# MarcBerliner/PETLION.jl

Hardware: AMD Instinct MI355X
Metric: DFN full-discharge trajectories/sec (ensemble) (higher is better)
Workload: dtype f64

## Files before the change

### petlion.jl_amd/csrc/dfn_cell.h

```cpp
#pragma once
#include <hip/hip_runtime.h>
#include <type_traits>
#include "../../include/petlion_hip.h"

namespace pl {

#ifndef PL_DEV
#define PL_DEV __device__ inline
#endif

constexpr int WAVE = 64;
#ifndef PL_NP
#define PL_NP 10
#endif
#ifndef PL_NS
#define PL_NS 10
#endif
#ifndef PL_NN
#define PL_NN 10
#endif
#ifndef PL_NR
#define PL_NR 10
#endif
#ifndef PL_NRN
// ... 275 lines not shown
#elif defined(PL_PHASE_FENCES) && !defined(PL_PHASE_TIMERS) && !defined(PL_WAVE_EMU)
#define PL_FENCE_() __asm__ volatile("" ::: "memory")
#define PL_AMARK(txt) PL_FENCE_()
#define PL_TIC() PL_FENCE_()
#define PL_TOC(S_, ph) PL_FENCE_()
#define PL_TIC_TOTAL() do {} while (0)
#define PL_TOC_TOTAL(S_) do {} while (0)
#define PL_TICD() PL_FENCE_()
#define PL_TOCD(S_, slot) PL_FENCE_()
#define PL_TICE(mode) PL_FENCE_()
#define PL_TOCE(S_, mode, slot) PL_FENCE_()
#else
#define PL_TIC() PL_TIC_()
#define PL_TOC(S_, ph) PL_TOC_(S_, ph)
#define PL_TIC_TOTAL() do {} while (0)
#define PL_TOC_TOTAL(S_) PL_TOC_(S_, PH_TOTAL)
#define PL_TICD() do {} while (0)
#define PL_TOCD(S_, slot) do {} while (0)
#define PL_TICE(mode) do {} while (0)
#define PL_TOCE(S_, mode, slot) do {} while (0)
#endif
#ifndef PL_AMARK
#define PL_AMARK(txt) do {} while (0)
#endif
__host__ __device__ __forceinline__ int sec_of(int i) { return i < NP ? 0 : (i < NP + NS ? 1 : 2); }
#ifndef PL_WAVE_EMU
template <int CTRL> __device__ __forceinline__ double dpp_mov0(double v) {
  int lo = __double2loint(v), hi = __double2hiint(v);
  lo = __builtin_amdgcn_update_dpp(0, lo, CTRL, 0xf, 0xf, true);
  hi = __builtin_amdgcn_update_dpp(0, hi, CTRL, 0xf, 0xf, true);
  return __hiloint2double(hi, lo);
}
__device__ __forceinline__ double shift_up1(double v) { return dpp_mov0<0x138>(v); }
__device__ __forceinline__ double shift_down1(double v) { return dpp_mov0<0x130>(v); }
__device__ __forceinline__ double row_up2(double v) { return dpp_mov0<0x112>(v); }
__device__ __forceinline__ double row_down2(double v) { return dpp_mov0<0x102>(v); }
__device__ __forceinline__ double lane_bcast(double v, int src) {
  const int lo = __builtin_amdgcn_readlane(__double2loint(v), src), hi = __builtin_amdgcn_readlane(__double2hiint(v), src);
  return __hiloint2double(hi, lo);
}
__device__ __forceinline__ int lane_bcast_i(int v, int src) { return __builtin_amdgcn_readlane(v, src); }
__device__ __forceinline__ double wave_sum(double v) {
  v += dpp_mov0<0x111>(v); v += dpp_mov0<0x112>(v); v += dpp_mov0<0x114>(v); v += dpp_mov0<0x118>(v);
  return (lane_bcast(v, 15) + lane_bcast(v, 31)) + (lane_bcast(v, 47) + lane_bcast(v, 63));
}
#else
// ... 1429 lines not shown
```

### petlion.jl_amd/csrc/dfn_integrate.h

```cpp
#pragma once
#include "dfn_cell.h"

namespace pl {

constexpr int NTRIP_MAX = (2 * NE + NJ * NR + 2 * NJ + 1 + (NT > 2 * NN + 1 ? NT : 2 * NN + 1) + WAVE - 1) / WAVE;
struct IdaScalars {
  double tn, hh, hused, cj, cjlast, cjold, cjratio, ss, rr, h0_forced, rtol, atol;
  double ew[NTRIP_MAX];
  double ph[4][NTRIP_MAX];
  double ee[NTRIP_MAX];
  double pa[NTRIP_MAX], pb[NTRIP_MAX];
  int kk, kused, knew, phase, ns, maxord;
  int nst;
};

enum GenFlag { GF_STOPS = 1, GF_FUNC = 2, GF_EXPR = 4, GF_REFINE = 8, GF_GENROW = 16, GF_SENS = 32 };

enum Cnt { C_STEPS, C_RES, C_JAC, C_FACT, C_SOLVE, C_NEWTON, C_ERRFAIL, C_CONVFAIL, C_SUMKP2, C_INIT };
struct Counters { int v[10]; };
__device__ __forceinline__ void cnt_add(Counters& c, int k, int v = 1) { c.v[k] += v; }

#define PHI_RD(j, n) ((M::PHI_LDS > MAXORD || (j) < M::PHI_LDS) ? S.phi[(M::PHI_LDS > MAXORD || (j) < M::PHI_LDS) ? (j) : 0][n] : ((j) == M::PHI_LDS ? I.ph[0][k__] : ((j) == M::PHI_LDS + 1 ? I.ph[1][k__] : ((j) == M::PHI_LDS + 2 ? I.ph[2][k__] : I.ph[3][k__]))))
#define PHI_WR(j, n, v) do { if (M::PHI_LDS > MAXORD || (j) < M::PHI_LDS) S.phi[(M::PHI_LDS > MAXORD || (j) < M::PHI_LDS) ? (j) : 0][n] = (v); \
                           else if ((j) == M::PHI_LDS) I.ph[0][k__] = (v); else if ((j) == M::PHI_LDS + 1) I.ph[1][k__] = (v); \
                           else if ((j) == M::PHI_LDS + 2) I.ph[2][k__] = (v); else I.ph[3][k__] = (v); } while (0)
#define EE(n) I.ee[k__]
template <class M> constexpr bool PHI_REGS = M::PHI_LDS <= MAXORD;
#ifdef PL_EXP_BRANCHY_PHI
constexpr bool PL_BRANCHY_PHI = true;
#else
constexpr bool PL_BRANCHY_PHI = false;
#endif
template <class M> constexpr bool PL_FLAT = M::PHI_LDS > MAXORD && !M::W2;
#define PL_VEC(n) _Pragma("unroll") for (int k__ = 0; k__ < NTRIP; k__++) if (const int n = vrow<M>(k__, lane, wave_id()); vok<M>(k__, lane, wave_id()))
#define PL_VECG(n) _Pragma("unroll") for (int k__ = 0; k__ < NTRIP; k__++) if (const int n = vrow<M>(k__, lane, wave_id()); vokg<M>(k__, lane, wave_id()))

template <class M>
__device__ __forceinline__ double wrms(const double* v, const double* w) {
  PL_MODEL(M);
  const int lane = lane_id();
  double s = 0.0;
  PL_VEC(n) { const double p = v[n] * w[n]; s += p * p; }
  return sqrt(wave_sum(s) * (1.0 / NST));
}

PL_DEV double tab_eval(const plh_run& r, double t) {
  const int n = r.n_tab; const double* tt = r.tab_t; const double* vv = r.tab_v;
  if (n <= 0) return 0.0;
  if (t < tt[0]) return vv[0];
  int lo = 0, hi = n;
  while (hi - lo > 1) { const int mid = (lo + hi) >> 1; if (tt[mid] <= t) lo = mid; else hi = mid; }
  const int k = lo;
  if (k == n - 1) return vv[n - 1];
  const double dt = tt[k + 1] - tt[k];
  return dt > 0.0 ? vv[k] + (vv[k + 1] - vv[k]) * ((t - tt[k]) / dt) : vv[k + 1];
}
// ... 317 lines not shown
  PL_XSYNC();
  PL_AMARK("form_iterate end");
}

template <int F, class M>
PL_DEV int ida_nls(CellLDS<M>& S, LaneRegs& R, const Tables* tb, IdaScalars& I, int mode, double value, int jac_every_step, Counters& cnt, int nref, const plh_run* xrun = nullptr,
                   double* xvalue = nullptr, GenRow* g = nullptr) {
  PL_MODEL(M);
  const int lane = lane_id();
  const double epsNewt = 0.33, toldel = 0.0001 * epsNewt;
  int callLSetup = 0;
  if (I.nst == 0) { I.cjold = I.cj; I.ss = 20.0; callLSetup = 1; }
  else {
    I.cjratio = pl_div(I.cj, I.cjold);
    const double temp1 = (1.0 - 0.25) / (1.0 + 0.25), temp2 = 1.0 / temp1;
    if (I.cjratio < temp1 || I.cjratio > temp2) callLSetup = 1;
    if (I.cj != I.cjlast) I.ss = 100.0;
    if (jac_every_step) callLSetup = 1;
  }
  PL_VEC(n) EE(n) = 0.0;
  PL_SYNC();
  int jcur = 0, ret = 0, m = 0; bool done = false; double oldnrm = 0.0;
  for (bool first = true;; first = false) {
    { PL_TIC(); form_iterate(S, I, first); PL_TOC(S, PH_NEWTVEC); }
    if (done) break;
    if constexpr ((F & GF_EXPR) != 0) { if (xrun) { value = closure_input(S, *xrun, I.tn, S.yy, S.yp); *xvalue = value; } }
    if (callLSetup) {
      PL_TIC();
      cell_res_jac(S, R, S.yy, S.yp, S.delta, mode, value);
      bool genf = false;
      if constexpr ((F & GF_GENROW) != 0) { if (g && g->on()) { genf = true; gen_factor(S, R, tb, I.cj, mode, false, *g, I.tn, S.yy, S.yp, S.yp); } }
      if (!genf) cell_factor(S, R, tb, I.cj, mode, false);
      cnt_add(cnt, C_RES); cnt_add(cnt, C_JAC); cnt_add(cnt, C_FACT);
      I.cjold = I.cj; I.cjratio = 1.0; I.ss = 20.0; jcur = 1; callLSetup = 0;
      PL_TOC(S, PH_JACFACT);
    } else {
      PL_TIC();
      cell_residual(S, R, S.yy, S.yp, S.delta, mode, value);
      cnt_add(cnt, C_RES);
      PL_TOC(S, PH_RES);
    }
    cnt_add(cnt, C_NEWTON); cnt_add(cnt, C_SOLVE);
    { PL_TIC();
    bool gens = false;
    if constexpr ((F & GF_GENROW) != 0) gens = g && g->on();
    if ((F & GF_REFINE) && nref > 0) cell_solve_refined(S, R, tb, S.delta, S.yp, I.cjold, mode, false, nref, gens ? g : nullptr);
// ... 70 lines not shown
    if (kk > 2) {
      const double enorm_km2 = pl_sqrt(s2 * (1.0 / NST)); const double err_km2 = sg_km2 * enorm_km2; const double terr_km2 = (kk - 1) * err_km2;
      if ((terr_km1 > terr_km2 ? terr_km1 : terr_km2) <= terr_k) I.knew = kk - 1;
    } else if (terr_km1 <= 0.5 * terr_k) I.knew = kk - 1;
  }
  PL_AMARK("test_error end");
  return (ck * enorm_k > 1.0) ? 1 : 0;
}

template <class M>
PL_DEV void ida_restore(CellLDS<M>& S, IdaScalars& I, double saved_t) {
  PL_MODEL(M);
  const int lane = lane_id();
  I.tn = saved_t;
  if (lane == 0 && wave_id() == 0) for (int j = 1; j <= I.kk; j++) S.ida_psi[j - 1] = S.ida_psi[j] - I.hh;
  if constexpr (PHI_REGS<M>) {
    _Pragma("unroll") for (int j = 0; j <= MAXORD; j++) if (j >= I.ns && j <= I.kk) { const double b = 1.0 / S.ida_beta[j]; PL_VEC(n) PHI_WR(j, n, PHI_RD(j, n) * b); }
  } else {
    if (I.ns <= I.kk) for (int j = I.ns; j <= I.kk; j++) { const double b = 1.0 / S.ida_beta[j]; PL_VEC(n) PHI_WR(j, n, PHI_RD(j, n) * b); }
  }
  PL_XSYNC();
}

template <class M>
PL_DEV bool ida_complete_step(CellLDS<M>& S, IdaScalars& I, double err_k, double err_km1, double tstop) {
  PL_MODEL(M);
  const int lane = lane_id();
  PL_AMARK("complete_step");
  I.nst++;
  const int kdiff = I.kk - I.kused; I.kused = I.kk; I.hused = I.hh;
  if (I.knew == I.kk - 1 || I.kk == I.maxord) I.phase = 1;
  if (I.phase == 0) { if (I.nst > 1) { I.kk++; I.hh *= 2.0; } }
  else {
    int action = 0;
    double err_kp1 = 0.0, err_knew;
    if (I.knew == I.kk - 1) action = 1;
    else if (I.kk == I.maxord) action = 2;
    else if (I.kk + 1 >= I.ns || kdiff == 1) action = 2;
    if (action == 0) {
      double s = 0.0;
      if constexpr (PHI_REGS<M>) {
        _Pragma("unroll") for (int j = 2; j <= MAXORD; j++) if (j == I.kk + 1) { PL_VEC(n) { const double p = (EE(n) - PHI_RD(j, n)) * EWT(n); s += p * p; } }
      } else { PL_VEC(n) { const double p = (EE(n) - PHI_RD(I.kk + 1, n)) * EWT(n); s += p * p; } }
      const double enorm = pl_sqrt(block_sum<M>(S, s) * (1.0 / NST)); err_kp1 = pl_div(enorm, (double)(I.kk + 2));
      const double terr_k = (I.kk + 1) * err_k, terr_kp1 = (I.kk + 2) * err_kp1;
      if (I.kk == 1) action = (terr_kp1 >= 0.5 * terr_k) ? 2 : 3;
      else { const double terr_km1 = I.kk * err_km1;
        if (terr_km1 <= (terr_k < terr_kp1 ? terr_k : terr_kp1)) action = 1; else if (terr_kp1 >= terr_k) action = 2; else action = 3; }
// ... 28 lines not shown
      (void)dku;
      const bool grow = ku < I.maxord;
      PL_VEC(n) { acc[k__] = EE(n); sp[k__] = 0.0; }
      if (ku >= 3) {
        double q5[NTRIP], q4[NTRIP];
        PL_VEC(n) { q5[k__] = S.phi[5][n]; q4[k__] = S.phi[4][n]; }
        const double m5 = ku >= 5 ? 1.0 : 0.0, m4 = ku >= 4 ? 1.0 : 0.0;
        PL_VEC(n) { acc[k__] += m5 * q5[k__]; q5[k__] = acc[k__]; sp[k__] += dc5 * acc[k__]; acc[k__] += m4 * q4[k__]; q4[k__] = acc[k__]; sp[k__] += dc4 * acc[k__]; }
        if (ku >= 5) { PL_VEC(n) S.phi[5][n] = q5[k__]; } else if (grow && ku == 4) { PL_VEC(n) S.phi[5][n] = EE(n); }
        if (ku >= 4) { PL_VEC(n) S.phi[4][n] = q4[k__]; } else if (grow) { PL_VEC(n) S.phi[4][n] = EE(n); }
      }
      double q[4][NTRIP];
      _Pragma("unroll") for (int j = 3; j >= 0; j--) PL_VEC(n) q[j][k__] = S.phi[j][n];
      const double m3 = ku >= 3 ? 1.0 : 0.0, m2 = ku >= 2 ? 1.0 : 0.0;
      PL_VEC(n) {
        acc[k__] += m3 * q[3][k__]; q[3][k__] = acc[k__]; sp[k__] += dc3 * acc[k__];
        acc[k__] += m2 * q[2][k__]; q[2][k__] = acc[k__]; sp[k__] += dc2 * acc[k__];
        acc[k__] += q[1][k__]; q[1][k__] = acc[k__]; sp[k__] += dc1 * acc[k__];
        acc[k__] += q[0][k__];
      }
      if (ku >= 3) { PL_VEC(n) S.phi[3][n] = q[3][k__]; } else if (grow && ku == 2) { PL_VEC(n) S.phi[3][n] = EE(n); }
      if (ku >= 2) { PL_VEC(n) S.phi[2][n] = q[2][k__]; } else if (grow) { PL_VEC(n) S.phi[2][n] = EE(n); }
      PL_VEC(n) { S.phi[1][n] = q[1][k__]; S.phi[0][n] = acc[k__]; }
    } else if constexpr (PHI_REGS<M> && PL_BRANCHY_PHI) {
      _Pragma("unroll") for (int j = MAXORD; j >= 0; j--) {
        if (j == ku + 1 && ku < I.maxord) { PL_VEC(n) PHI_WR(j, n, EE(n)); }
        else if (j == ku) { PL_VEC(n) { acc[k__] = PHI_RD(j, n) + EE(n); PHI_WR(j, n, acc[k__]); sp[k__] = dku * acc[k__]; } }
        else if (j < ku) {
          const double dj = j == 1 ? dc1 : j == 2 ? dc2 : j == 3 ? dc3 : j == 4 ? dc4 : 0.0;
          PL_VEC(n) { acc[k__] += PHI_RD(j, n); PHI_WR(j, n, acc[k__]); if (j > 0) sp[k__] += dj * acc[k__]; }
        }
      }
    } else if constexpr (PHI_REGS<M>) {
      (void)dku;
      const bool grow = ku < I.maxord;
      PL_VEC(n) { acc[k__] = EE(n); sp[k__] = 0.0; }
      _Pragma("unroll") for (int j = MAXORD; j >= 0; j--) {
        const double dj = j == 1 ? dc1 : j == 2 ? dc2 : j == 3 ? dc3 : j == 4 ? dc4 : j == 5 ? dc5 : 0.0;
        if (j < M::PHI_LDS) {
          PL_VEC(n) { acc[k__] += S.phi[j][n]; S.phi[j][n] = acc[k__]; if (j > 0) sp[k__] += dj * acc[k__]; }
        } else {
          const bool in = j <= ku, take_ee = grow && j == ku + 1;
          const double m = in ? 1.0 : 0.0;
          PL_VEC(n) {
            const double ph = PHI_RD(j, n), e = EE(n);
            const double an = acc[k__] + m * ph;
// ... 43 lines not shown
  PL_XSYNC();
}

PL_DEV double next_tstop(const plh_opts& o, double t, bool continuation, double tf) {
  double best = tf;
  if (continuation && 1.0 > t && 1.0 < best) best = 1.0;
  if (o.n_tstops > 0) {
    const double lim = t > 0.0 ? t : 0.0;
    int lo = -1, hi = o.n_tstops;
    while (hi - lo > 1) { const int mid = (lo + hi) >> 1; if (o.tstops[mid] > lim) hi = mid; else lo = mid; }
    if (hi < o.n_tstops && o.tstops[hi] < best) best = o.tstops[hi];
  }
  if (o.n_tdiscon > 0) {
    const double lim = (t > 0.0 ? t : 0.0) + o.reltol / 2;
    int lo = -1, hi = o.n_tdiscon;
    while (hi - lo > 1) { const int mid = (lo + hi) >> 1; if (o.tdiscon[mid] > lim) hi = mid; else lo = mid; }
    for (int q = hi > 0 ? hi - 1 : 0; q < o.n_tdiscon; q++) { const double s = o.tdiscon[q] - o.reltol / 2; if (s > t && s > 0.0) { if (s < best) best = s; break; } }
  }
  return best;
}

template <int F, class M>
PL_DEV int ida_step(CellLDS<M>& S, LaneRegs& R, const Tables* tb, IdaScalars& I, double tstop, double& tret, int mode, double& value,
                               const plh_opts& o, Counters& cnt, const plh_run* frun = nullptr, GenRow* g = nullptr) {
  PL_MODEL(M);
  const int lane = lane_id();
  const double uround = 2.220446049250313e-16;
  I.rtol = o.reltol; I.atol = o.abstol;
  if (I.nst == 0) {
    set_ewt(S, I, o.reltol, o.abstol);
    const double tdist = fabs(tstop - I.tn);
    double hh = I.h0_forced != 0.0 ? I.h0_forced : o.init_step;
    if (hh == 0.0) {
      hh = 0.001 * tdist;
      double sy = 0.0;
      PL_VEC(n) { const double pq = S.phi[1][n] * EWT(n); sy += pq * pq; }
      const double ypnorm = sqrt(block_sum<M>(S, sy) * (1.0 / NST));
      if (ypnorm > 0.5 / hh) hh = 0.5 / ypnorm;
    }
    if ((I.tn + hh - tstop) * hh > 0.0) hh = (tstop - I.tn) * (1.0 - 4.0 * uround);
    I.hh = hh; I.kk = 0; I.kused = 0;
    PL_VEC(n) S.phi[1][n] *= hh;
    PL_SYNC();
  } else {
    const double troundoff = 100.0 * uround * (fabs(I.tn) + fabs(I.hh));
    if (fabs(I.tn - tstop) <= troundoff) { ida_get_solution(S, I, tstop, S.yy, S.yp); tret = tstop; return 0; }
    if ((I.tn + I.hh - tstop) * I.hh > 0.0) I.hh = (tstop - I.tn) * (1.0 - 4.0 * uround);
    set_ewt(S, I, o.reltol, o.abstol);
  }
  const double saved_t = I.tn; int ncf = 0, nef = 0; double err_k = 0, err_km1 = 0;
  if (I.nst == 0) { I.kk = 1; I.kused = 0; I.hused = 0.0; if (lane == 0 && wave_id() == 0) S.ida_psi[0] = I.hh; I.cj = 1.0 / I.hh; I.phase = 0; I.ns = 0; PL_XSYNC(); }
  for (;;) {
    double ck; { PL_TIC(); PL_TICE(3); ck = ida_set_coeffs(S, I); PL_TOC(S, PH_STEPCTL); PL_TOCE(S, 3, 0); }
    if constexpr ((F & GF_FUNC) != 0) { if (frun && frun->mode != PLH_MODE_DSTATE) value = run_input<F>(S, *frun, I.tn, S.yy, S.yp); }
    const int nflag = ida_nls<F>(S, R, tb, I, mode, value, o.jac_every_step, cnt, o.refine, ((F & GF_EXPR) && frun && (frun->value_kind == PLH_VAL_EXPR || frun->mode == PLH_MODE_DSTATE)) ? frun : nullptr, &value, g);
    int errfail = 0;
    if (nflag == 0) { PL_TIC(); PL_TICE(3); errfail = ida_test_error(S, I, ck, err_k, err_km1); PL_TOC(S, PH_STEPCTL); PL_TOCE(S, 3, 1); }
    if (nflag != 0 || errfail) {
      ida_restore(S, I, saved_t);
      I.phase = 1;
      if (!errfail) {
        cnt_add(cnt, C_CONVFAIL);
        I.rr = 0.25; I.hh *= I.rr; ncf++;
        if (ncf >= 10) return PLH_ERR_STALL;
      } else {
        cnt_add(cnt, C_ERRFAIL); nef++;
        if (nef == 1) { const double err_knew = (I.kk == I.knew) ? err_k : err_km1; I.kk = I.knew;
          I.rr = 0.9 * pl_inv_root(2.0 * err_knew + 0.0001, I.kk + 1); I.rr = I.rr < 0.9 ? I.rr : 0.9; I.rr = I.rr > 0.25 ? I.rr : 0.25; I.hh *= I.rr; }
        else if (nef == 2) { I.kk = I.knew; I.rr = 0.25; I.hh *= I.rr; }
        else if (nef < 10) { I.kk = 1; I.rr = 0.25; I.hh *= I.rr; }
        else return PLH_ERR_STALL;
      }
      const double tscale = fabs(I.tn) > 1.0 ? fabs(I.tn) : 1.0;
      if (fabs(I.hh) < 1e-14 * tscale) return PLH_ERR_STALL;
      if (I.nst == 0) { if (lane == 0 && wave_id() == 0) S.ida_psi[0] = I.hh; const double rr = I.rr; PL_VEC(n) S.phi[1][n] *= rr; PL_XSYNC(); }
      continue;
    }
    break;
  }
  cnt_add(cnt, C_STEPS); cnt_add(cnt, C_SUMKP2, I.kk + 2);
#ifdef PL_WAVE_EMU
  if (getenv("PL_EMU_TRACE") && lane == 0 && blockIdx.x == 0) fprintf(stderr, "dev step %d tn %.9g h %.6g k %d knew %d phase %d ns %d err_k %.6e err_km1 %.6e nef %d ncf %d\n", I.nst + 1, I.tn, I.hh, I.kk, I.knew, I.phase, I.ns, err_k, err_km1, nef, ncf);
#endif
  PL_TIC(); PL_TICE(3);
  const bool have_sol = ida_complete_step(S, I, err_k, err_km1, tstop);
  PL_TOCE(S, 3, 2);
  if (!have_sol) { ida_get_solution(S, I, tstop, S.yy, S.yp); tret = tstop; PL_TOC(S, PH_STEPCTL); PL_TOCE(S, 3, 3); return 0; }
  if ((I.tn + I.hh - tstop) * I.hh > 0.0) I.hh = (tstop - I.tn) * (1.0 - 4.0 * uround);
  tret = I.tn;
  PL_TOC(S, PH_STEPCTL); PL_TOCE(S, 3, 3);
  return 0;
}

struct PrevVals { double frac, V, SOC, I, c_s_n, c_e_min, eta_pl, dfilm, T, g; };

template <class M>
__device__ __forceinline__ double cellV(const double* Y) { return Y[M::O_PS] - Y[M::O_PS + NJ - 1]; }

template <class M>
__device__ __forceinline__ double cellTavg(const CellLDS<M>& S, const double* Y) {
  if constexpr (M::THERMAL) { const int lane = lane_id(); return wave_sum(lane < NT ? S.th.wT5[tsec_of(lane)] * Y[M::O_T + lane] : 0.0); }
  else return S.cc.T0;
}

template <int F = 0, class M>
PL_DEV void check_stop(CellLDS<M>& S, const plh_run& run, const plh_opts& o, double t, double tf, const double* Y, const double* YP,
                                  double SOC, PrevVals& pv, int& flag) {
  PL_MODEL(M);
  const double eps = t < 1.0 ? o.reltol : 0.0;
  [[maybe_unused]] double Tav = 0.0, dTav = 0.0;
  if constexpr (M::THERMAL) { Tav = cellTavg<M>(S, Y); dTav = cellTavg<M>(S, YP); }
  const plh_bounds& b = run.bounds;
  double bImax = b.I_max, bImin = b.I_min, bVmin = b.V_min, bVmax = b.V_max, bSmin = b.SOC_min, bSmax = b.SOC_max, bcs = b.c_s_n_max, bce = b.c_e_min;
  double bep = b.eta_plating_min, Ic = Y[O_I], dI = YP[O_I], V = cellV<M>(Y), dV = cellV<M>(YP), ep = Y[O_PS + NP] - Y[O_PE + NP + NS], dep = YP[O_PS + NP] - YP[O_PE + NP + NS];
  [[maybe_unused]] double bTmax = M::THERMAL ? b.T_max : 0.0;
  const int rmode = run.mode, vkind = run.value_kind;
  pl_pin(bImax, bImin, bVmin, bVmax, bSmin, bSmax, bcs, bce); pl_pin(bep, Ic, dI, V, dV, ep, dep, bTmax);
  if (t >= tf) { flag = 0; return; }
  if (!o.check_bounds || vkind == PLH_VAL_REST) return;
  if (rmode != PLH_MODE_I) {
    if ((Ic - bImax > eps) && dI > 0) { const double f = (pv.I - bImax) / (pv.I - Ic); if (f < pv.frac) { pv.frac = f; flag = 7; } }
    else if ((bImin - Ic > eps) && dI < 0) { const double f = (pv.I - bImin) / (pv.I - Ic); if (f < pv.frac) { pv.frac = f; flag = 8; } }
    pv.I = Ic;
  }
  if (rmode != PLH_MODE_V) {
    if ((bVmin - V > eps) && dV < 0) { const double f = (pv.V - bVmin) / (pv.V - V); if (f < pv.frac) { pv.frac = f; flag = 1; } }
    else if ((V - bVmax > eps) && dV > 0) { const double f = (pv.V - bVmax) / (pv.V - V); if (f < pv.frac) { pv.frac = f; flag = 2; } }
    pv.V = V;
  }
  {
    if ((bSmin - SOC > eps) && Ic < 0) { const double f = (pv.SOC - bSmin) / (pv.SOC - SOC); if (f < pv.frac) { pv.frac = f; flag = 3; } }
    else if ((SOC - bSmax > eps) && Ic > 0) { const double f = (pv.SOC - bSmax) / (pv.SOC - SOC); if (f < pv.frac) { pv.frac = f; flag = 4; } }
    pv.SOC = SOC;
  }
  if constexpr (M::THERMAL) {
    if (bTmax == bTmax && rmode != PLH_MODE_DT) {
      if (Tav - bTmax > eps && dTav > 0) { const double f = (pv.T - bTmax) / (pv.T - Tav); if (f < pv.frac) { pv.frac = f; flag = 5; } }
// ... 52 lines not shown
  bool have_prev = false;
  const double T0 = S.cc.T0;
  if (Yinit && !from_states) {
    PL_VECG(n) S.yy[n] = Yinit[n];
    PL_XSYNC();
    have_prev = true;
    if (lane == 0 && wave_id() == 0) { S.carry[0] = SOC0; S.carry[1] = t_init; S.carry[2] = cellV<M>(S.yy); S.carry[3] = S.yy[O_I]; S.carry[4] = S.yy[O_PS + NP] - S.yy[O_PE + NP + NS]; }
  } else {
    if (Yinit) { PL_VECG(n) S.yy[n] = Yinit[n]; PL_XSYNC(); }
    if (lane == 0 && wave_id() == 0) { S.carry[0] = SOC0; S.carry[1] = 0.0; S.carry[2] = 0.0; S.carry[3] = 0.0; S.carry[4] = 0.0; }
  }
  PL_XSYNC();
  double* const outp = wave_id() != 0 ? nullptr : (lane == 0 ? out.t : (lane == 1 ? out.V : (lane == 2 ? out.I : (lane == 3 ? out.SOC : (lane == 4 ? out.T : nullptr)))));
  auto save_pt = [&](int idx, double tt, const double* Y, double soc) {
    const double Tav = (M::THERMAL && out.T) ? cellTavg<M>(S, Y) : T0;
    if constexpr ((F & GF_STOPS) != 0) if (out.Yall && idx < out.max_pts) { PL_VECG(n) out.Yall[(size_t)idx * NST + n] = Y[n]; }
    if constexpr ((F & GF_STOPS) != 0) if (out.Ysel && idx < out.max_pts) {
      double* const row = out.Ysel + (size_t)idx * out.sel_tot;
      for (int k = lane + WAVE * wave_id(); k < out.sel_tot; k += WAVE * M::NWAVES) row[k] = Y[out.sel_map[k]];
    }
    double Vv = cellV<M>(Y), Iv = Y[O_I];
    pl_pin(Vv, Iv);
    const double val = lane == 0 ? tt : (lane == 1 ? Vv : (lane == 2 ? Iv : (lane == 3 ? soc : Tav)));
    if (outp && idx < out.max_pts) outp[idx] = val;
  };
  for (int r = 0; r < n_runs; r++) {
    PL_XSYNC();
    if (lane == 0 && wave_id() == 0) { S.runc = runs[r]; if (S.runc.value_cell) S.runc.value = S.runc.value_cell[cell]; if (S.runc.tf_cell) S.runc.tf = S.runc.tf_cell[cell]; }
    PL_XSYNC();
    const plh_run& run = S.runc;
    double SOC = S.carry[0];
    const double t_global = S.carry[1], prev_V = S.carry[2], prev_I = S.carry[3], prev_etap = S.carry[4];
    const bool dstate = (F & GF_GENROW) && run.mode == PLH_MODE_DSTATE;
    const int mode = dstate ? PLH_MODE_RES : run.mode;
    if constexpr ((F & GF_GENROW) != 0) {
      if (dstate) {
        const int kind = run.dstate;
        const int first = kind <= PLH_DSTATE_CS_P_MIN ? O_CS + (M::SD == 0 ? cs_surf(0) : 0) : (kind <= PLH_DSTATE_CS_N_MIN ? O_CS + (M::SD == 0 ? cs_surf(NP) : NP) : O_CE);
        const int count = kind <= PLH_DSTATE_CS_P_MIN ? NP : (kind <= PLH_DSTATE_CS_N_MIN ? NN : NE);
        const int stride = M::SD != 0 ? 1 : (kind <= PLH_DSTATE_CS_P_MIN ? NRP : (kind <= PLH_DSTATE_CS_N_MIN ? NRN : 1));
        const bool want_max = (kind & 1) != 0;
        int best = first; double bv = S.yy[first];
        for (int q = 1; q < count; q++) { const double v = S.yy[first + q * stride]; if (want_max ? v > bv : v < bv) { bv = v; best = first + q * stride; } }
        PL_XSYNC();
        if (lane == 0 && wave_id() == 0) S.runc.dstate = best;
        PL_XSYNC();
// ... 29 lines not shown
    } else if (mode == PLH_MODE_P) {
      if (run.value_kind == PLH_VAL_HOLD) { value = prev_I * S.cc.I1C * prev_V; Iguess = prev_I; }
      else if (run.value_kind == PLH_VAL_REST) { value = 0.0; Iguess = 0.0; }
      else Iguess = value / (cellV<M>(S.yy) * S.cc.I1C);
    } else if (mode == PLH_MODE_ETA_P) {
      if (run.value_kind == PLH_VAL_HOLD) { value = prev_etap; Iguess = prev_I; }
      else if (have_prev) Iguess = prev_I;
      else { const double OCV = cellV<M>(S.yy); Iguess = value > OCV ? 1.0 : -1.0; }
    } else {
      if (run.value_kind == PLH_VAL_HOLD) value = 0.0;
      Iguess = have_prev ? prev_I : 1.0;
    }
    PL_XSYNC();
    if (lane == 0 && wave_id() == 0) S.yy[O_I] = Iguess;
    PL_XSYNC();
    GenRow grow;
    if constexpr ((F & GF_GENROW) != 0) { if (((run.value_kind == PLH_VAL_EXPR && run.n_dcol > 0) || dstate) && genW) { grow.run = &run; grow.W = genW; } }
    int flag = PLH_FLAG_RUNNING;
    plh_run_info ri; ri.flag = PLH_FLAG_RUNNING; ri.iterations = 0; ri.t_end = t_global; ri.V = 0; ri.I = 0; ri.SOC = SOC; ri.T_avg = T0;
    const bool continuation = !new_run;
    PrevVals pv; pv.frac = 1.0; pv.V = -1; pv.SOC = -1; pv.I = -1; pv.c_s_n = -1; pv.c_e_min = -1; pv.eta_pl = -1; pv.dfilm = -1; pv.T = -1; pv.g = -1;
    double tprev = 0.0, t = 0.0, t_prev_saved = t0; int iter = 1; bool stalled_once = false;
    double I_prev_pt = 0.0, t_restart = 0.0;
    [[maybe_unused]] double soc_nm1_s = 0.0, dt_step_s = 0.0, soc_n_s = 0.0;
    bool first_init = true, again = false, init_failed = false;
    [[maybe_unused]] int steps_since_restart = 2;
    auto init_block = [&]() -> bool {
    again = false;
    int ierr; { PL_TIC(); ierr = cell_init_consistent<F>(S, R, tb, S.yy, S.yp, S.delta, S.phi[1], mode, value, o.reltol_init, cnt, S.phi[0], o.refine,
                                                                       ((F & GF_EXPR) && (run.value_kind == PLH_VAL_EXPR || dstate)) ? &run : nullptr, t_restart, &grow); PL_TOC(S, PH_INIT); }
    if (ierr != 0) { if (first_init) init_failed = true; else flag = ierr; ri.flag = ierr; return false; }
    if constexpr ((F & GF_STOPS) != 0) { if (o.yp_alg_zero) { PL_VEC(n) if (n >= NDIFF) S.yp[n] = 0.0; PL_XSYNC(); } }
    ida_reinit(S, I, S.yy, S.yp, first_init ? (o.max_order > 0 && o.max_order <= MAXORD ? o.max_order : MAXORD) : I.maxord, t_restart);
    if (first_init) {
      first_init = false;
      save_pt(nout, t0, S.yy, SOC); nout++;
      check_stop<F>(S, run, o, 0.0, run.tf, S.yy, S.yp, SOC, pv, flag);
      PL_VECG(n) { Yprev[n] = S.yy[n]; YPprev[n] = S.yp[n]; }
      PL_SYNC();
      I_prev_pt = S.yy[O_I];
      if constexpr ((F & GF_SENS) != 0) sens_init(S, SX, mode, value, new_run, SOC0, o.reltol, o.abstol, nout - 1, run.value_kind == PLH_VAL_HOLD && have_prev, prev_V, prev_I);
    }
    return true;
    };
    bool init_ok = true;
    [[maybe_unused]] bool need_init = true;
    if constexpr ((F & GF_FUNC) == 0) init_ok = init_block();
    while (init_ok && flag == PLH_FLAG_RUNNING) {
      if constexpr ((F & GF_FUNC) != 0) {
        if (need_init) { need_init = false; if (!init_block()) break; if (flag != PLH_FLAG_RUNNING) break; }
      }
      double tret = t; tprev = t;
      double tstop_now;
      if constexpr ((F & GF_STOPS) != 0) tstop_now = next_tstop(o, t, continuation, run.tf);
      else tstop_now = (continuation && run.tf > 1.0 && t < 1.0) ? 1.0 : run.tf;
      if constexpr (M::W2) __syncthreads();
      const int sf = ida_step<F>(S, R, tb, I, tstop_now, tret, mode, value, o, cnt, (is_tab || dstate) ? &run : nullptr, &grow);
      if (sf != 0) {
        if (I.nst == 0 && !stalled_once) {
          stalled_once = true;
          PL_VECG(n) { S.yy[n] = Yprev[n]; S.yp[n] = YPprev[n]; }
          PL_XSYNC();
          ida_reinit(S, I, S.yy, S.yp, I.maxord); I.h0_forced = o.reltol; iter++; t = tprev;
          save_pt(nout, t + t0, S.yy, SOC); nout++;
          if constexpr ((F & GF_SENS) != 0) sens_repeat_point(S, SX, nout - 1);
          check_stop<F>(S, run, o, t, run.tf, S.yy, S.yp, SOC, pv, flag);
          continue;
        }
        flag = sf; break;
      }
      iter++; t = tret;
      if constexpr ((F & GF_FUNC) != 0) steps_since_restart++;
      PL_TIC(); PL_TICE(3);
      const double SOC_new = SOC + pl_div(0.5 * ((t + t0) - t_prev_saved) * (S.yy[O_I] + I_prev_pt), 3600.0);
      [[maybe_unused]] const double dt_saved = (t + t0) - t_prev_saved, soc_before = SOC;
      if constexpr ((F & GF_SENS) != 0) { soc_nm1_s = soc_before; dt_step_s = dt_saved; }
      SOC = SOC_new;
      save_pt(nout, t + t0, S.yy, SOC); nout++;
      PL_TOCE(S, 3, 4);
      check_stop<F>(S, run, o, t, run.tf, S.yy, S.yp, SOC, pv, flag);
      PL_TOCE(S, 3, 5);
      if constexpr ((F & GF_SENS) != 0) sens_step(S, R, I, SX, mode, value, nout - 1, dt_saved);
      if (!is_fun && t == tprev) { flag = PLH_ERR_STALL; break; }
      if (iter == o.maxiters) { flag = PLH_ERR_MAXITERS; break; }
      if (nout >= out.max_pts && out.max_pts > 0 && flag == PLH_FLAG_RUNNING) { flag = PLH_ERR_OUTPUT_FULL; break; }
      if (flag == PLH_FLAG_RUNNING) {
        if (YPfin) { PL_VECG(n) YPprev[n] = S.yp[n]; }
        t_prev_saved = t + t0; I_prev_pt = S.yy[O_I];
        if constexpr ((F & GF_FUNC) != 0) if (is_fun && t - tprev < 1e-3 * o.reltol) {
          const double t_new = t + o.reltol, v_new = run_input<F>(S, run, t_new, S.yy, S.yp);
          const double big = fabs(value) > fabs(v_new) ? fabs(value) : fabs(v_new);
          const double tolv = o.abstol > o.reltol * big ? o.abstol : o.reltol * big;
          if (!(fabs(value - v_new) <= tolv)) {
            value = v_new; t_restart = t_new; again = true;
            PL_VECG(n) { Yprev[n] = S.yy[n]; YPprev[n] = S.yp[n]; }
            steps_since_restart = 0;
          }
        }
      }
      PL_TOC(S, PH_OUTPUT); PL_TOCE(S, 3, 6);
      if constexpr ((F & GF_FUNC) != 0) { if (again) need_init = true; }
    }
    if (init_failed) { if (lane == 0) info[r] = ri; for (int q = r + 1; q < n_runs; q++) if (lane == 0) { plh_run_info z = ri; z.flag = PLH_FLAG_RUNNING; info[q] = z; } break; }
    double t_end = t + t0;
    if constexpr ((F & GF_SENS) != 0) soc_n_s = SOC;
    if (flag > 0 && o.interp_final && t > 1.0) {
      const double fr = pv.frac;
      const double ti = fr * (t - tprev) + tprev;
      PL_XSYNC();
      if ((F & GF_FUNC) && steps_since_restart == 1) { PL_VECG(n) { const double yprev = Yprev[n]; S.yy[n] = fr * (S.yy[n] - yprev) + yprev; } }
      else { PL_VEC(n) { const double yprev = S.phi[0][n] - S.phi[1][n]; S.yy[n] = fr * (S.yy[n] - yprev) + yprev; } }
      if (YPfin) { PL_VECG(n) { const double ypp = YPprev[n]; S.yp[n] = fr * (S.yp[n] - ypp) + ypp; } }
      PL_XSYNC();
      SOC = SOC + 0.5 * ((ti + t0) - (t + t0)) * (S.yy[O_I] + S.yy[O_I]) / 3600.0;
      t_end = ti + t0;
      save_pt(nout - 1, t_end, S.yy, SOC);
    }
    if constexpr ((F & GF_SENS) != 0) sens_finish(S, SX, flag > 0 && o.interp_final && t > 1.0, pv.frac, flag < 0, nout - 1, flag, run.bounds, mode, soc_n_s, soc_nm1_s, dt_step_s, S.yy[O_I]);
    ri.flag = flag; ri.iterations = iter; ri.t_end = t_end; ri.V = cellV<M>(S.yy); ri.I = S.yy[O_I]; ri.SOC = SOC; ri.T_avg = cellTavg<M>(S, S.yy);
    if (lane == 0 && wave_id() == 0) info[r] = ri;
    have_prev = true;
    PL_XSYNC();
    if (lane == 0 && wave_id() == 0) { S.carry[0] = SOC; S.carry[1] = t_end; S.carry[2] = ri.V; S.carry[3] = ri.I; S.carry[4] = S.yy[O_PS + NP] - S.yy[O_PE + NP + NS]; }
// ... 12 lines not shown
```

### petlion.jl_amd/csrc/petlion_kernels.h

```cpp
#pragma once
#include "dfn_integrate.h"
#include "plh_host.h"

#ifndef PL_WAVE_EMU
#define PL_LAUNCH(kernel, grid, block, stream, ...) hipLaunchKernelGGL(kernel, dim3(grid), dim3(block), 0, stream, __VA_ARGS__)
#endif

namespace pl {

#ifndef PL_WAVE_EMU
#define PL_CELLS_PER_SIMD(M) ((sizeof(CellLDS<M>) <= 26624 && !M::W2) ? 2 : 1)
#define PL_ONE_WAVE_PER_SIMD __attribute__((amdgpu_waves_per_eu(M::NWAVES * PL_CELLS_PER_SIMD(M), M::NWAVES * PL_CELLS_PER_SIMD(M))))
#else
#define PL_ONE_WAVE_PER_SIMD
#endif

template <class M> __device__ __forceinline__ void load_vec(double* dst, const double* __restrict__ src) {
  const int lane = lane_id(), wv = wave_id();
  _Pragma("unroll") for (int k__ = 0; k__ < M::NTRIP; k__++) if (const int n = vrow<M>(k__, lane, wv); vokg<M>(k__, lane, wv)) dst[n] = src[n];
}
template <class M> __device__ __forceinline__ void store_vec(double* __restrict__ dst, const double* src) {
  const int lane = lane_id(), wv = wave_id();
  _Pragma("unroll") for (int k__ = 0; k__ < M::NTRIP; k__++) if (const int n = vrow<M>(k__, lane, wv); vokg<M>(k__, lane, wv)) dst[n] = src[n];
}

template <class M> __global__ __launch_bounds__(64 * M::NWAVES) PL_ONE_WAVE_PER_SIMD void k_initial_guess(const Tables* tb, int n_cells, const double* theta, const double* SOC, double* Y) {
  __shared__ CellLDS<M> S;
  PL_EMU_POISON(S);
  constexpr int NST = M::NST;
  LaneRegs R;
  const int cell = blockIdx.x;
  if (cell >= n_cells) return;
  cell_setup(S, R, tb, theta + (size_t)cell * tb->P);
  cell_initial_guess(S, S.yy, SOC[cell]);
// ... 306 lines not shown
```

Measured before the change: 956,000.

## Restructure step boundary to reuse register data and skip redundant work

For plain-flag kernels of large flat models, the error weights are now computed from the accepted solution still held in registers during step completion, and the separate ewt pass at the start of the next step is skipped. Output and stop-check scalars (current, voltage, plating overpotential) are broadcast from registers with readlane instead of being read back from LDS. The trailing form_iterate after Newton convergence is skipped and only recomputed on failure. This aims to cut LDS traffic and synchronisation at each step boundary, at the cost of extra special-case code paths.

Measured after the change: 966,400 (median of 6 runs). 1.1% higher.

```diff
diff --git a/petlion.jl_amd/csrc/dfn_cell.h b/petlion.jl_amd/csrc/dfn_cell.h
--- a/petlion.jl_amd/csrc/dfn_cell.h
+++ b/petlion.jl_amd/csrc/dfn_cell.h
@@ -321,6 +321,15 @@
 #endif
 #ifndef PL_AMARK
 #define PL_AMARK(txt) do {} while (0)
+#endif
+#if defined(PL_PHASE_TIMERS) && !defined(PL_WAVE_EMU) && defined(PL_PHASE_DETAIL) && PL_PHASE_DETAIL == 4
+#define PL_TICH(v) long long v = (long long)__builtin_readcyclecounter()
+#define PL_RETICH(v) v = (long long)__builtin_readcyclecounter()
+#define PL_TOCH(S_, v, slot) do { if (threadIdx.x == 0) (S_).cyc[slot] += (long long)__builtin_readcyclecounter() - v; } while (0)
+#else
+#define PL_TICH(v) do {} while (0)
+#define PL_RETICH(v) do {} while (0)
+#define PL_TOCH(S_, v, slot) do {} while (0)
 #endif
 __host__ __device__ __forceinline__ int sec_of(int i) { return i < NP ? 0 : (i < NP + NS ? 1 : 2); }
 #ifndef PL_WAVE_EMU
diff --git a/petlion.jl_amd/csrc/dfn_integrate.h b/petlion.jl_amd/csrc/dfn_integrate.h
--- a/petlion.jl_amd/csrc/dfn_integrate.h
+++ b/petlion.jl_amd/csrc/dfn_integrate.h
@@ -32,6 +32,31 @@
 constexpr bool PL_BRANCHY_PHI = false;
 #endif
 template <class M> constexpr bool PL_FLAT = M::PHI_LDS > MAXORD && !M::W2;
+#if defined(PL_OLD_STEP_BOUNDARY) && !defined(PL_WAVE_EMU) && !defined(PL_PHASE_TIMERS)
+#error "PL_OLD_STEP_BOUNDARY is for wave-emulator test builds and phase-timer profiling builds only"
+#endif
+constexpr size_t PL_TWO_CELLS_LDS_MAX = 26624;
+#ifdef PL_OLD_STEP_BOUNDARY
+template <int F, class M> constexpr bool PL_STEPB = false;
+#else
+template <int F, class M> constexpr bool PL_STEPB = F == 0 && PL_FLAT<M> && (sizeof(CellLDS<M>) > PL_TWO_CELLS_LDS_MAX);
+#endif
+struct StepPt { double I, dI, V, dV, ep, dep; };
+template <class M>
+__device__ __forceinline__ void step_pt_load(StepPt& pt, const double* Y, const double* YP) {
+  PL_MODEL(M);
+  pt.I = Y[O_I]; pt.dI = YP[O_I]; pt.V = Y[O_PS] - Y[O_PS + NJ - 1]; pt.dV = YP[O_PS] - YP[O_PS + NJ - 1];
+  pt.ep = Y[O_PS + NP] - Y[O_PE + NP + NS]; pt.dep = YP[O_PS + NP] - YP[O_PE + NP + NS];
+}
+#define PL_TRIP_BCAST(v, n) lane_bcast((v)[(n) / WAVE], (n) % WAVE)
+template <class M>
+__device__ __forceinline__ void step_pt_regs(StepPt& pt, const double* y, const double* yp) {
+  PL_MODEL(M);
+  static_assert(!M::W2, "entry n lives in trip n / 64 of lane n % 64 only with one wave per cell");
+  pt.I = PL_TRIP_BCAST(y, O_I); pt.dI = PL_TRIP_BCAST(yp, O_I);
+  pt.V = PL_TRIP_BCAST(y, O_PS) - PL_TRIP_BCAST(y, O_PS + NJ - 1); pt.dV = PL_TRIP_BCAST(yp, O_PS) - PL_TRIP_BCAST(yp, O_PS + NJ - 1);
+  pt.ep = PL_TRIP_BCAST(y, O_PS + NP) - PL_TRIP_BCAST(y, O_PE + NP + NS); pt.dep = PL_TRIP_BCAST(yp, O_PS + NP) - PL_TRIP_BCAST(yp, O_PE + NP + NS);
+}
 #define PL_VEC(n) _Pragma("unroll") for (int k__ = 0; k__ < NTRIP; k__++) if (const int n = vrow<M>(k__, lane, wave_id()); vok<M>(k__, lane, wave_id()))
 #define PL_VECG(n) _Pragma("unroll") for (int k__ = 0; k__ < NTRIP; k__++) if (const int n = vrow<M>(k__, lane, wave_id()); vokg<M>(k__, lane, wave_id()))
 
@@ -395,6 +420,7 @@
   PL_SYNC();
   int jcur = 0, ret = 0, m = 0; bool done = false; double oldnrm = 0.0;
   for (bool first = true;; first = false) {
+    if constexpr (PL_STEPB<F, M>) { if (done) break; }
     { PL_TIC(); form_iterate(S, I, first); PL_TOC(S, PH_NEWTVEC); }
     if (done) break;
     if constexpr ((F & GF_EXPR) != 0) { if (xrun) { value = closure_input(S, *xrun, I.tn, S.yy, S.yp); *xvalue = value; } }
@@ -511,8 +537,9 @@
   PL_XSYNC();
 }
 
-template <class M>
-PL_DEV bool ida_complete_step(CellLDS<M>& S, IdaScalars& I, double err_k, double err_km1, double tstop) {
+template <class M, bool SB = false>
+PL_DEV bool ida_complete_step(CellLDS<M>& S, IdaScalars& I, double err_k, double err_km1, double tstop, [[maybe_unused]] double rtol = 0.0, [[maybe_unused]] double atol = 0.0,
+                              [[maybe_unused]] StepPt* pt = nullptr) {
   PL_MODEL(M);
   const int lane = lane_id();
   PL_AMARK("complete_step");
@@ -587,6 +614,10 @@
       if (ku >= 3) { PL_VEC(n) S.phi[3][n] = q[3][k__]; } else if (grow && ku == 2) { PL_VEC(n) S.phi[3][n] = EE(n); }
       if (ku >= 2) { PL_VEC(n) S.phi[2][n] = q[2][k__]; } else if (grow) { PL_VEC(n) S.phi[2][n] = EE(n); }
       PL_VEC(n) { S.phi[1][n] = q[1][k__]; S.phi[0][n] = acc[k__]; }
+      if constexpr (SB) {
+        PL_VEC(n) { const double w = pl_rcp(rtol * fabs(acc[k__]) + atol); I.ew[k__] = w; }
+        step_pt_regs<M>(*pt, acc, sp);
+      }
     } else if constexpr (PHI_REGS<M> && PL_BRANCHY_PHI) {
       _Pragma("unroll") for (int j = MAXORD; j >= 0; j--) {
         if (j == ku + 1 && ku < I.maxord) { PL_VEC(n) PHI_WR(j, n, EE(n)); }
@@ -676,11 +707,12 @@
 
 template <int F, class M>
 PL_DEV int ida_step(CellLDS<M>& S, LaneRegs& R, const Tables* tb, IdaScalars& I, double tstop, double& tret, int mode, double& value,
-                               const plh_opts& o, Counters& cnt, const plh_run* frun = nullptr, GenRow* g = nullptr) {
+                               const plh_opts& o, Counters& cnt, const plh_run* frun = nullptr, GenRow* g = nullptr, [[maybe_unused]] StepPt* pt = nullptr) {
   PL_MODEL(M);
   const int lane = lane_id();
   const double uround = 2.220446049250313e-16;
   I.rtol = o.reltol; I.atol = o.abstol;
+  PL_TICH(pl_th__);
   if (I.nst == 0) {
     set_ewt(S, I, o.reltol, o.abstol);
     const double tdist = fabs(tstop - I.tn);
@@ -698,12 +730,17 @@
     PL_SYNC();
   } else {
     const double troundoff = 100.0 * uround * (fabs(I.tn) + fabs(I.hh));
-    if (fabs(I.tn - tstop) <= troundoff) { ida_get_solution(S, I, tstop, S.yy, S.yp); tret = tstop; return 0; }
+    if (fabs(I.tn - tstop) <= troundoff) {
+      ida_get_solution(S, I, tstop, S.yy, S.yp); tret = tstop;
+      if constexpr (PL_STEPB<F, M>) step_pt_load<M>(*pt, S.yy, S.yp);
+      return 0;
+    }
     if ((I.tn + I.hh - tstop) * I.hh > 0.0) I.hh = (tstop - I.tn) * (1.0 - 4.0 * uround);
-    set_ewt(S, I, o.reltol, o.abstol);
+    if constexpr (!PL_STEPB<F, M>) set_ewt(S, I, o.reltol, o.abstol);
   }
   const double saved_t = I.tn; int ncf = 0, nef = 0; double err_k = 0, err_km1 = 0;
   if (I.nst == 0) { I.kk = 1; I.kused = 0; I.hused = 0.0; if (lane == 0 && wave_id() == 0) S.ida_psi[0] = I.hh; I.cj = 1.0 / I.hh; I.phase = 0; I.ns = 0; PL_XSYNC(); }
+  PL_TOCH(S, pl_th__, 0);
   for (;;) {
     double ck; { PL_TIC(); PL_TICE(3); ck = ida_set_coeffs(S, I); PL_TOC(S, PH_STEPCTL); PL_TOCE(S, 3, 0); }
     if constexpr ((F & GF_FUNC) != 0) { if (frun && frun->mode != PLH_MODE_DSTATE) value = run_input<F>(S, *frun, I.tn, S.yy, S.yp); }
@@ -737,9 +774,13 @@
   if (getenv("PL_EMU_TRACE") && lane == 0 && blockIdx.x == 0) fprintf(stderr, "dev step %d tn %.9g h %.6g k %d knew %d phase %d ns %d err_k %.6e err_km1 %.6e nef %d ncf %d\n", I.nst + 1, I.tn, I.hh, I.kk, I.knew, I.phase, I.ns, err_k, err_km1, nef, ncf);
 #endif
   PL_TIC(); PL_TICE(3);
-  const bool have_sol = ida_complete_step(S, I, err_k, err_km1, tstop);
+  const bool have_sol = ida_complete_step<M, PL_STEPB<F, M>>(S, I, err_k, err_km1, tstop, o.reltol, o.abstol, pt);
   PL_TOCE(S, 3, 2);
-  if (!have_sol) { ida_get_solution(S, I, tstop, S.yy, S.yp); tret = tstop; PL_TOC(S, PH_STEPCTL); PL_TOCE(S, 3, 3); return 0; }
+  if (!have_sol) {
+    ida_get_solution(S, I, tstop, S.yy, S.yp); tret = tstop;
+    if constexpr (PL_STEPB<F, M>) step_pt_load<M>(*pt, S.yy, S.yp);
+    PL_TOC(S, PH_STEPCTL); PL_TOCE(S, 3, 3); return 0;
+  }
   if ((I.tn + I.hh - tstop) * I.hh > 0.0) I.hh = (tstop - I.tn) * (1.0 - 4.0 * uround);
   tret = I.tn;
   PL_TOC(S, PH_STEPCTL); PL_TOCE(S, 3, 3);
@@ -759,14 +800,16 @@
 
 template <int F = 0, class M>
 PL_DEV void check_stop(CellLDS<M>& S, const plh_run& run, const plh_opts& o, double t, double tf, const double* Y, const double* YP,
-                                  double SOC, PrevVals& pv, int& flag) {
+                                  double SOC, PrevVals& pv, int& flag, [[maybe_unused]] const StepPt* pt = nullptr) {
   PL_MODEL(M);
   const double eps = t < 1.0 ? o.reltol : 0.0;
   [[maybe_unused]] double Tav = 0.0, dTav = 0.0;
   if constexpr (M::THERMAL) { Tav = cellTavg<M>(S, Y); dTav = cellTavg<M>(S, YP); }
   const plh_bounds& b = run.bounds;
   double bImax = b.I_max, bImin = b.I_min, bVmin = b.V_min, bVmax = b.V_max, bSmin = b.SOC_min, bSmax = b.SOC_max, bcs = b.c_s_n_max, bce = b.c_e_min;
-  double bep = b.eta_plating_min, Ic = Y[O_I], dI = YP[O_I], V = cellV<M>(Y), dV = cellV<M>(YP), ep = Y[O_PS + NP] - Y[O_PE + NP + NS], dep = YP[O_PS + NP] - YP[O_PE + NP + NS];
+  double bep = b.eta_plating_min, Ic, dI, V, dV, ep, dep;
+  if (PL_STEPB<F, M> && pt) { Ic = pt->I; dI = pt->dI; V = pt->V; dV = pt->dV; ep = pt->ep; dep = pt->dep; }
+  else { Ic = Y[O_I]; dI = YP[O_I]; V = cellV<M>(Y); dV = cellV<M>(YP); ep = Y[O_PS + NP] - Y[O_PE + NP + NS]; dep = YP[O_PS + NP] - YP[O_PE + NP + NS]; }
   [[maybe_unused]] double bTmax = M::THERMAL ? b.T_max : 0.0;
   const int rmode = run.mode, vkind = run.value_kind;
   pl_pin(bImax, bImin, bVmin, bVmax, bSmin, bSmax, bcs, bce); pl_pin(bep, Ic, dI, V, dV, ep, dep, bTmax);
@@ -865,6 +908,10 @@
     double Vv = cellV<M>(Y), Iv = Y[O_I];
     pl_pin(Vv, Iv);
     const double val = lane == 0 ? tt : (lane == 1 ? Vv : (lane == 2 ? Iv : (lane == 3 ? soc : Tav)));
+    if (outp && idx < out.max_pts) outp[idx] = val;
+  };
+  [[maybe_unused]] auto save_pt_regs = [&](int idx, double tt, const StepPt& pt, double soc) {
+    const double val = lane == 0 ? tt : (lane == 1 ? pt.V : (lane == 2 ? pt.I : (lane == 3 ? soc : T0)));
     if (outp && idx < out.max_pts) outp[idx] = val;
   };
   for (int r = 0; r < n_runs; r++) {
@@ -940,6 +987,10 @@
     PrevVals pv; pv.frac = 1.0; pv.V = -1; pv.SOC = -1; pv.I = -1; pv.c_s_n = -1; pv.c_e_min = -1; pv.eta_pl = -1; pv.dfilm = -1; pv.T = -1; pv.g = -1;
     double tprev = 0.0, t = 0.0, t_prev_saved = t0; int iter = 1; bool stalled_once = false;
     double I_prev_pt = 0.0, t_restart = 0.0;
+    [[maybe_unused]] StepPt spt;
+#if defined(PL_WAVE_EMU) && !defined(PL_OLD_STEP_BOUNDARY)
+    static_assert(!(F == 0 && PL_FLAT<M> && M::NST >= 301) || PL_STEPB<F, M>, "emulator build: the plain kernel of a 301-state model must take the new step boundary");
+#endif
     [[maybe_unused]] double soc_nm1_s = 0.0, dt_step_s = 0.0, soc_n_s = 0.0;
     bool first_init = true, again = false, init_failed = false;
     [[maybe_unused]] int steps_since_restart = 2;
@@ -964,6 +1015,7 @@
     bool init_ok = true;
     [[maybe_unused]] bool need_init = true;
     if constexpr ((F & GF_FUNC) == 0) init_ok = init_block();
+    PL_TICH(pl_tl__);
     while (init_ok && flag == PLH_FLAG_RUNNING) {
       if constexpr ((F & GF_FUNC) != 0) {
         if (need_init) { need_init = false; if (!init_block()) break; if (flag != PLH_FLAG_RUNNING) break; }
@@ -973,7 +1025,8 @@
       if constexpr ((F & GF_STOPS) != 0) tstop_now = next_tstop(o, t, continuation, run.tf);
       else tstop_now = (continuation && run.tf > 1.0 && t < 1.0) ? 1.0 : run.tf;
       if constexpr (M::W2) __syncthreads();
-      const int sf = ida_step<F>(S, R, tb, I, tstop_now, tret, mode, value, o, cnt, (is_tab || dstate) ? &run : nullptr, &grow);
+      PL_TOCH(S, pl_tl__, 1);
+      const int sf = ida_step<F>(S, R, tb, I, tstop_now, tret, mode, value, o, cnt, (is_tab || dstate) ? &run : nullptr, &grow, &spt);
       if (sf != 0) {
         if (I.nst == 0 && !stalled_once) {
           stalled_once = true;
@@ -985,18 +1038,23 @@
           check_stop<F>(S, run, o, t, run.tf, S.yy, S.yp, SOC, pv, flag);
           continue;
         }
+        if constexpr (PL_STEPB<F, M>) { static_assert(!PL_STEPB<F, M> || M::PRED_REGS, "the predictor of the last attempt must still be in registers"); form_iterate(S, I, false); }
         flag = sf; break;
       }
       iter++; t = tret;
       if constexpr ((F & GF_FUNC) != 0) steps_since_restart++;
       PL_TIC(); PL_TICE(3);
-      const double SOC_new = SOC + pl_div(0.5 * ((t + t0) - t_prev_saved) * (S.yy[O_I] + I_prev_pt), 3600.0);
+      double I_pt;
+      if constexpr (PL_STEPB<F, M>) I_pt = spt.I; else I_pt = S.yy[O_I];
+      const double SOC_new = SOC + pl_div(0.5 * ((t + t0) - t_prev_saved) * (I_pt + I_prev_pt), 3600.0);
       [[maybe_unused]] const double dt_saved = (t + t0) - t_prev_saved, soc_before = SOC;
       if constexpr ((F & GF_SENS) != 0) { soc_nm1_s = soc_before; dt_step_s = dt_saved; }
       SOC = SOC_new;
-      save_pt(nout, t + t0, S.yy, SOC); nout++;
+      if constexpr (PL_STEPB<F, M>) save_pt_regs(nout, t + t0, spt, SOC); else save_pt(nout, t + t0, S.yy, SOC);
+      nout++;
       PL_TOCE(S, 3, 4);
-      check_stop<F>(S, run, o, t, run.tf, S.yy, S.yp, SOC, pv, flag);
+      if constexpr (PL_STEPB<F, M>) check_stop<F>(S, run, o, t, run.tf, S.yy, S.yp, SOC, pv, flag, &spt);
+      else check_stop<F>(S, run, o, t, run.tf, S.yy, S.yp, SOC, pv, flag);
       PL_TOCE(S, 3, 5);
       if constexpr ((F & GF_SENS) != 0) sens_step(S, R, I, SX, mode, value, nout - 1, dt_saved);
       if (!is_fun && t == tprev) { flag = PLH_ERR_STALL; break; }
@@ -1004,7 +1062,8 @@
       if (nout >= out.max_pts && out.max_pts > 0 && flag == PLH_FLAG_RUNNING) { flag = PLH_ERR_OUTPUT_FULL; break; }
       if (flag == PLH_FLAG_RUNNING) {
         if (YPfin) { PL_VECG(n) YPprev[n] = S.yp[n]; }
-        t_prev_saved = t + t0; I_prev_pt = S.yy[O_I];
+        t_prev_saved = t + t0;
+        if constexpr (PL_STEPB<F, M>) I_prev_pt = spt.I; else I_prev_pt = S.yy[O_I];
         if constexpr ((F & GF_FUNC) != 0) if (is_fun && t - tprev < 1e-3 * o.reltol) {
           const double t_new = t + o.reltol, v_new = run_input<F>(S, run, t_new, S.yy, S.yp);
           const double big = fabs(value) > fabs(v_new) ? fabs(value) : fabs(v_new);
@@ -1017,6 +1076,7 @@
         }
       }
       PL_TOC(S, PH_OUTPUT); PL_TOCE(S, 3, 6);
+      PL_RETICH(pl_tl__);
       if constexpr ((F & GF_FUNC) != 0) { if (again) need_init = true; }
     }
     if (init_failed) { if (lane == 0) info[r] = ri; for (int q = r + 1; q < n_runs; q++) if (lane == 0) { plh_run_info z = ri; z.flag = PLH_FLAG_RUNNING; info[q] = z; } break; }
diff --git a/petlion.jl_amd/csrc/petlion_kernels.h b/petlion.jl_amd/csrc/petlion_kernels.h
--- a/petlion.jl_amd/csrc/petlion_kernels.h
+++ b/petlion.jl_amd/csrc/petlion_kernels.h
@@ -9,7 +9,7 @@
 namespace pl {
 
 #ifndef PL_WAVE_EMU
-#define PL_CELLS_PER_SIMD(M) ((sizeof(CellLDS<M>) <= 26624 && !M::W2) ? 2 : 1)
+#define PL_CELLS_PER_SIMD(M) ((sizeof(CellLDS<M>) <= PL_TWO_CELLS_LDS_MAX && !M::W2) ? 2 : 1)
 #define PL_ONE_WAVE_PER_SIMD __attribute__((amdgpu_waves_per_eu(M::NWAVES * PL_CELLS_PER_SIMD(M), M::NWAVES * PL_CELLS_PER_SIMD(M))))
 #else
 #define PL_ONE_WAVE_PER_SIMD
```
